# mj129/Tramba

Hardware: AMD Instinct MI355X
Metric: images/sec fwd Tramba-V 384x384 (higher is better)
Workload: dtype bf16; 1 GPU; Tramba-V (VMamba-B encoder) 384x384 bf16 inference, batch 4 per GPU, random-init weights (seed 1026), randn images; global_batch=4, launch=hipGraph replay, decoder guide branches on a side stream

## Files before the change

### include/tramba_hip.h

```cpp
#ifndef TRAMBA_HIP_H
#define TRAMBA_HIP_H

#include <stddef.h>
#include <stdint.h>

#ifdef __cplusplus
extern "C" {
#endif

typedef enum { TRAMBA_F32 = 0, TRAMBA_F16 = 1, TRAMBA_BF16 = 2 } tramba_dtype;

typedef enum {
    TRAMBA_SCAN_RASTER = 0,
    TRAMBA_SCAN_LINE = 1,
    TRAMBA_SCAN_HELIX = 2,
    TRAMBA_SCAN_WINDOW = 3,
    TRAMBA_SCAN_DILATION = 4
} tramba_scan_family;

typedef enum { TRAMBA_ACT_NONE = 0, TRAMBA_ACT_SILU = 1, TRAMBA_ACT_GELU = 2,
               TRAMBA_ACT_SIGMOID_GATE = 3 ,
               TRAMBA_ACT_GELU_GRAD_MUL = 4
             } tramba_act;

// ... 133 lines not shown
                     int64_t m, int n, int k, int act, int dtype, int out_dtype, void *stream);
int tramba_linear_ln_cl(const void *x, const void *w_folded, const float *colsum, const float *bias, const void *residual,
                        void *y, int64_t m, int n, int k, float eps, int act, int dtype, int out_dtype, void *stream);
int tramba_linear2_cl(const void *x1, const void *x2, int k1, const void *w, const float *bias, const void *residual,
                      void *y, int64_t m, int n, int k, int act, int dtype, int out_dtype, void *stream);

int tramba_linear_dual_cl(const void *x, const void *w, const float *bias, void *y_pre, void *y_act, int64_t m, int n,
                          int k, int act, int dtype, void *stream);
size_t tramba_wgrad_workspace(int64_t m, int n, int k, int groups, int nbatch);
int tramba_wgrad_cl(const void *gy, const void *x, float *out, void *workspace, size_t workspace_bytes, int64_t m, int n,
                    int k, int groups, int nbatch, int64_t gy_bs, int64_t gy_gs, int gy_ld, int64_t x_bs, int64_t x_gs,
                    int x_ld, int want_bias, int dtype, void *stream);
int tramba_wgrad_parts_cl(const void *gy, const void *x, float *out, void *workspace, size_t workspace_bytes, int64_t m,
                          int n, int k, int groups, int nbatch, int64_t gy_bs, int64_t gy_gs, int gy_ld, int64_t x_bs,
                          int64_t x_gs, int x_ld, int want_bias, int dtype, void *stream, int *nslab);
int tramba_rows_gemm_cl(const void *x, const void *w, float *y, int nz, int64_t m, int n, int k, int groups, int ldy,
                        int dtype, void *stream);
int tramba_shadow_cast_multi(const void *table, int ntensors, int64_t total_tiles, int dtype, void *stream);
int tramba_slab_sum(const float *part, float *out, int64_t n, int nslab, void *stream);
int tramba_multi_sum_strided(const float *const *parts, float *const *outs, const int64_t *n, const int64_t *stride,
                             const int *nslab, int count, void *stream);
int tramba_multi_sum(const float *const *parts, float *const *outs, const int64_t *n, const int *nslab, int count,
                     void *stream);

int tramba_expand_norm_head_cl(const void *x, const void *w, const float *ln_w, const float *ln_b,
                               const float *head_w, float head_b, float *y, int batch, int h, int wd, int cin, int p,
                               float eps, int dtype, void *stream);

int tramba_conv3x3s2_cl(const void *x, const void *w, const float *bias, void *y, int batch, int hin,
                        int win, int cin, int cout, int dtype, void *stream);
int tramba_stem_conv_ln_gelu(const void *img, const float *w, const float *bias, const float *ln_w,
                             const float *ln_b, void *y, int batch, int h, int wd, float eps,
                             int img_dtype, int dtype, void *stream);

#define TRAMBA_EVAL_NINT 520
#define TRAMBA_EVAL_NDBL 48
int tramba_saliency_stats(const float *pred, const unsigned char *gt, long long *ints, double *dbl, int batch, int h,
                          int w, void *stream);
#define TRAMBA_WFM_MAX_DIM 4096
int tramba_feature_transform(const unsigned char *gt, int *idx, int *dist2, int batch, int h, int w, void *stream);
size_t tramba_weighted_f_workspace(int batch, int h, int w);
int tramba_weighted_f_sums(const float *pred, const unsigned char *gt, const int *idx, const int *dist2, const double *gauss,
                           double *sums, void *workspace, size_t workspace_bytes, int batch, int h, int w, void *stream);

#define TRAMBA_FRAME_MAX_DIM 16384
#define TRAMBA_FRAME_MAX_OUT 2048
size_t tramba_resize_table_words(int in_h, int in_w, int out_h, int out_w);
int tramba_resize_table(int in_h, int in_w, int out_h, int out_w, const double *mean, const double *std, int *table,
                        size_t words);
int tramba_frames_to_input(const unsigned char *frames, const int *table, float *out, int batch, int h, int w, int out_h,
                           int out_w, int bgr, void *stream);
int tramba_logits_to_u8(const void *logits, unsigned char *out, int batch, int in_h, int in_w, int h, int w, int dtype,
                        void *stream);
#define TRAMBA_FRAMES_DESC_WORDS 16
#define TRAMBA_RAGGED_IN 1
#define TRAMBA_RAGGED_OUT 2
int tramba_frames_ragged_check(const int64_t *desc_host, int batch, int size, size_t packed_bytes, size_t out_capacity,
                               int parts);
int tramba_frames_to_input_ragged(const unsigned char *packed, const int64_t *desc_host, size_t packed_bytes, float *out,
                                  int batch, int size, int bgr, void *stream);
int tramba_logits_to_u8_ragged(const void *logits, const unsigned char *packed, const int64_t *desc_host, unsigned char *out,
                               size_t out_capacity, int batch, int size, int dtype, void *stream);

#define TRAMBA_AUG_DESC_WORDS 32
#define TRAMBA_AUG_CONTRAST 0
#define TRAMBA_AUG_BRIGHTNESS 1
// ... 102 lines not shown
```

### tramba_amd/csrc/norm_conv.hip

```cpp
#include <stdlib.h>
#include <string.h>

#include "common.h"
#include "norm.h"

namespace tramba {

template <typename T, int V>
__global__ __launch_bounds__(256) void layernorm_cl_kernel(const T *__restrict__ x,
                                                          const float *__restrict__ w,
                                                          const float *__restrict__ bvec, T *__restrict__ y,
                                                          long rows, int C, float eps, int act, int P, int H,
                                                          int W)
{
    const int lane = threadIdx.x & (kWave - 1);
    const long row = (long)blockIdx.x * (blockDim.x >> 6) + __builtin_amdgcn_readfirstlane(threadIdx.x >> 6);
    if (row >= rows) return;
    const int nit = (C + kWave * V - 1) / (kWave * V);
    float acc[kNormMaxIt][V];
    const T *xr = x + row * C;
#pragma unroll
    for (int it = 0; it < kNormMaxIt; ++it) {
#pragma unroll
        for (int v = 0; v < V; ++v) acc[it][v] = 0.f;
// ... 1033 lines not shown
                    dw_v2f p[TW];
#pragma unroll
                    for (int t = 0; t < TW; ++t) {
                        p[t] = acc[u % KS][t];
                        acc[u % KS][t] = bias;
                    }
                    if constexpr (DUAL) {
#pragma unroll
                        for (int t = 0; t < TW; ++t) {
                            dw_store2<T>(rp, voff[t + R], so, p[t]);
                            p[t] = dw_v2f{Cvt<T>::to_f(Cvt<T>::from_f(p[t].x)), Cvt<T>::to_f(Cvt<T>::from_f(p[t].y))};
                        }
                    }
                    if (act == TRAMBA_ACT_GELU) {
#pragma unroll
                        for (int t = 0; t < TW; ++t) p[t] = dw_v2f{geluf_(p[t].x), geluf_(p[t].y)};
                    } else if (act == TRAMBA_ACT_SILU) {
#pragma unroll
                        for (int t = 0; t < TW; ++t) p[t] = dw_v2f{siluf_(p[t].x), siluf_(p[t].y)};
                    }
#pragma unroll
                    for (int t = 0; t < TW; ++t) dw_store2<T>(ry, voff[t + R], so, p[t]);
                }
                issue(q + D < nq ? r + D : -1, swr);
                srd = srd + 1 == NS ? 0 : srd + 1;
                swr = swr + 1 == NS ? 0 : swr + 1;
            }
        }
    }
    asm volatile("s_waitcnt vmcnt(0)" ::: "memory");
#endif
}

template <typename T>
__device__ __forceinline__ dw_v2f dw_load2(__amdgpu_buffer_rsrc_t r, unsigned voff)
{
    if constexpr (sizeof(T) == 4) {
        return __builtin_bit_cast(dw_v2f, __builtin_amdgcn_raw_buffer_load_b64(r, voff, 0, 0));
    } else {
        const unsigned raw = __builtin_amdgcn_raw_buffer_load_b32(r, voff, 0, 0);
        const Pack<T, 2> pk = __builtin_bit_cast(Pack<T, 2>, raw);
        return dw_v2f{Cvt<T>::to_f(pk.v[0]), Cvt<T>::to_f(pk.v[1])};
    }
}

constexpr int dwg_waves(int ks) { return ks <= 3 ? 16 : 8; }

template <typename T, int KS>
__global__ __launch_bounds__(dwg_waves(KS) * kWave) void dwconv_wgrad_cl_kernel(const T *__restrict__ x,
                                                                          const T *__restrict__ gy,
                                                                          float *__restrict__ part, int H, int W, int C,
                                                                          int RPW, int CS)
{
    constexpr int V = 2, R = KS / 2, TW = 4, NI = TW + KS - 1, kDwgWaves = dwg_waves(KS);
    __shared__ float red[KS * KS + 1][2 * kWave];
    const int lane = threadIdx.x & (kWave - 1);
    const int wv = __builtin_amdgcn_readfirstlane(threadIdx.x >> 6);
    const int c0 = (blockIdx.x * kWave + lane) * V;
    const bool cok = c0 + V <= C;
    const int band = blockIdx.y / CS, cs = blockIdx.y % CS;
    const int row0 = (band * kDwgWaves + wv) * RPW;
    const int wseg = ((W + CS - 1) / CS + TW - 1) / TW * TW;
    const int wlo = cs * wseg, whi = wlo + wseg < W ? wlo + wseg : W;
    const int b = blockIdx.z;
    const unsigned colb = (unsigned)C * (unsigned)sizeof(T), rowb = (unsigned)W * colb;
    const __amdgpu_buffer_rsrc_t rx = make_rsrc(x + (long)b * H * W * C, (unsigned)H * rowb);
// ... 254 lines not shown
    return TRAMBA_OK;
}

static int dw7_band_rows(long items4, int H)
{
    const int cand[] = {6, 8, 12, 16, 24, 32, 48, 64, 96, 128, 192};
    int best = H;
    double best_cost = 1e30;
    for (int th : cand) {
        if (th > H && th != cand[0]) continue;
        const int t = th > H ? H : th;
        const long nwg = items4 * ((H + t - 1) / t);
        const double cost = (double)((nwg + 255) / 256) * (t * 196.0 + (t + 6) * 50.0 + 150.0);
        if (cost < best_cost) { best_cost = cost; best = t; }
    }
    return best;
}

template <typename T>
static int launch_dw7_march(const void *x, const float *wt, const float *bt, void *y, int B, int H, int W, int C, int act,
                            hipStream_t s, void *ypre, int flip)
{
    const int nct = (C / 2 + 63) / 64, ncg = (W + kDwmTW - 1) / kDwmTW;
    const long items4 = ((long)nct * ncg * B + 3) / 4;
    int th = dw7_band_rows(items4, H);
    const int forced = tramba_tune_get(TRAMBA_TUNE_DW_ROWS);
    if (forced > 0) th = forced > H ? H : forced;
    const int nbands = (H + th - 1) / th;
    if (ypre)
        hipLaunchKernelGGL((dwconv7_march_kernel<T, true>), dim3((unsigned)(items4 * nbands)), dim3(256), 0, s, (const T *)x, wt, bt,
                           (T *)y, B, H, W, C, act, (T *)ypre, flip, th, nbands, nct, ncg);
    else
        hipLaunchKernelGGL((dwconv7_march_kernel<T, false>), dim3((unsigned)(items4 * nbands)), dim3(256), 0, s, (const T *)x, wt, bt,
                           (T *)y, B, H, W, C, act, (T *)ypre, flip, th, nbands, nct, ncg);
    TRAMBA_LAUNCH_CHECK();
    return TRAMBA_OK;
}

}

using namespace tramba;

extern "C" int tramba_layernorm_cl(const void *x, const float *w, const float *b, void *y, int64_t rows,
                                   int c, float eps, int act, int dtype, void *stream)
{
    TRAMBA_CHECK(x && w && b && y, "layernorm_cl: null tensor");
    TRAMBA_CHECK(rows > 0 && c > 0, "layernorm_cl: empty shape");
    TRAMBA_CHECK(aligned16(x) && aligned16(y), "layernorm_cl: tensors must be 16-byte aligned");
    ProfScope prof(TRAMBA_PROF_LAYERNORM, (hipStream_t)stream, 2.0 * (double)rows * c * dtype_size(dtype));
    TRAMBA_DISPATCH_DTYPE(dtype, T,
        return launch_layernorm<T>(x, w, b, y, rows, c, eps, act, 1, 1, 1, (hipStream_t)stream));
    return TRAMBA_OK;
}

static long ln_bwd_rows_per_wave(long rows, bool rows_form)
{
    long rpw = rows / 4096;
    const long lo = rows_form ? 4 : 2;
    return rpw < lo ? lo : (rpw > 128 ? 128 : rpw);
}

static bool ln_bwd_rows_form(int c, int dtype)
{
    const int vm = dtype == TRAMBA_F32 ? 4 : 8;
    return c % vm == 0 && c <= kWave * vm;
}
// ... 451 lines not shown
        constexpr int VM = 16 / (int)sizeof(T);
        if (vec) {
            const long total = pixels * (c / VM);
            hipLaunchKernelGGL((col2im3x3_cl_kernel<T, VM>), dim3((unsigned)((total + 255) / 256)), dim3(256), 0, s,
                               (const T *)gcols, (T *)gx, h, wd, c, ho, wo, stride, pad, ckp, total);
        } else {
            const long total = pixels * c;
            hipLaunchKernelGGL((col2im3x3_cl_kernel<T, 1>), dim3((unsigned)((total + 255) / 256)), dim3(256), 0, s,
                               (const T *)gcols, (T *)gx, h, wd, c, ho, wo, stride, pad, ckp, total);
        }
    });
    TRAMBA_LAUNCH_CHECK();
    return TRAMBA_OK;
}

extern "C" int tramba_dwconv_cl(const void *x, const float *wt, const float *bt, void *y, int batch, int h,
                                int wd, int c, int ks, int act, int dtype, void *stream)
{
    return tramba_dwconv_dual_cl(x, wt, bt, nullptr, y, batch, h, wd, c, ks, act, 0, dtype, stream);
}

extern "C" int tramba_dwconv_dual_cl(const void *x, const float *wt, const float *bt, void *y_pre, void *y, int batch,
                                     int h, int wd, int c, int ks, int act, int flip_taps, int dtype, void *stream)
{
    TRAMBA_CHECK(x && wt && bt && y, "dwconv_cl: null tensor");
    TRAMBA_CHECK(!y_pre || aligned16(y_pre), "dwconv_cl: tensors must be 16-byte aligned");
    TRAMBA_CHECK(batch > 0 && h > 0 && wd > 0 && c > 0, "dwconv_cl: empty shape");
    TRAMBA_CHECK(ks == 3 || ks == 5 || ks == 7, "dwconv_cl: kernel size %d unsupported (3,5,7)", ks);
    TRAMBA_CHECK(aligned16(x) && aligned16(y) && aligned16(wt) && aligned16(bt), "dwconv_cl: tensors must be 16-byte aligned");
    hipStream_t s = (hipStream_t)stream;
    ProfScope prof(TRAMBA_PROF_DW, s, (y_pre ? 3.0 : 2.0) * (double)batch * h * wd * c * dtype_size(dtype));
    const bool march = ks == 7 && c % 8 == 0 && tramba_tune_get(TRAMBA_TUNE_DW_FORM) != 1 &&
                       (double)h * wd * c * 4.0 < 2147483648.0 && (double)batch * wd * c < 2147483648.0;
    TRAMBA_DISPATCH_DTYPE(dtype, T, {
        if (march) return launch_dw7_march<T>(x, wt, bt, y, batch, h, wd, c, act, s, y_pre, flip_taps);
        if (ks == 3) return launch_dw<T, 3>(x, wt, bt, y, batch, h, wd, c, act, s, y_pre, flip_taps);
        if (ks == 5) return launch_dw<T, 5>(x, wt, bt, y, batch, h, wd, c, act, s, y_pre, flip_taps);
        return launch_dw<T, 7>(x, wt, bt, y, batch, h, wd, c, act, s, y_pre, flip_taps);
    });
    return TRAMBA_OK;
}
```

### tramba_amd/csrc/stem.hip

```cpp
#include "common.h"

namespace tramba {

constexpr int kStemCout = 64, kStemTaps = 27;

template <typename TI, typename T>
__global__ __launch_bounds__(256) void stem_conv_ln_gelu_kernel(const TI *__restrict__ img, const float *__restrict__ w,
                                                               const float *__restrict__ bias,
                                                               const float *__restrict__ ln_w,
                                                               const float *__restrict__ ln_b, T *__restrict__ y,
                                                               int B, int H, int W, int Ho, int Wo, float eps)
{
    __shared__ __attribute__((aligned(16))) float wl[kStemTaps][kStemCout];
    for (int t = threadIdx.x; t < kStemTaps * kStemCout; t += blockDim.x) {
        const int co = t / kStemTaps, tap = t % kStemTaps;
        wl[tap][co] = w[t];
    }
    __syncthreads();
    const long pix = (long)blockIdx.x * 64 + (threadIdx.x >> 2);
    const int part = threadIdx.x & 3;
    const long npix = (long)B * Ho * Wo;
    const bool ok = pix < npix;
    const long pp = ok ? pix : npix - 1;
    const int wo = (int)(pp % Wo);
    const long t2 = pp / Wo;
    const int ho = (int)(t2 % Ho), b = (int)(t2 / Ho);

    float acc[16];
#pragma unroll
    for (int j = 0; j < 16; ++j) acc[j] = bias[part * 16 + j];
#pragma unroll 1
    for (int ci = 0; ci < 3; ++ci)
#pragma unroll 1
        for (int ky = 0; ky < 3; ++ky) {
            const int hy = 2 * ho + ky - 1;
#pragma unroll
            for (int kx = 0; kx < 3; ++kx) {
                const int wx = 2 * wo + kx - 1;
                float v = 0.f;
                if (hy >= 0 && hy < H && wx >= 0 && wx < W) v = Cvt<TI>::to_f(img[(((long)b * 3 + ci) * H + hy) * W + wx]);
                const float4 *wp = reinterpret_cast<const float4 *>(&wl[ci * 9 + ky * 3 + kx][part * 16]);
#pragma unroll
                for (int q = 0; q < 4; ++q) {
                    const float4 ww = wp[q];
                    acc[4 * q + 0] = fmaf(v, ww.x, acc[4 * q + 0]);
                    acc[4 * q + 1] = fmaf(v, ww.y, acc[4 * q + 1]);
                    acc[4 * q + 2] = fmaf(v, ww.z, acc[4 * q + 2]);
                    acc[4 * q + 3] = fmaf(v, ww.w, acc[4 * q + 3]);
                }
            }
        }
    float s = 0.f;
#pragma unroll
    for (int j = 0; j < 16; ++j) s += acc[j];
    s += __shfl_xor(s, 1, 4);
    s += __shfl_xor(s, 2, 4);
    const float mean = s * (1.f / kStemCout);
    float q2 = 0.f;
#pragma unroll
    for (int j = 0; j < 16; ++j) {
        const float d = acc[j] - mean;
        q2 = fmaf(d, d, q2);
    }
    q2 += __shfl_xor(q2, 1, 4);
    q2 += __shfl_xor(q2, 2, 4);
    const float rstd = rsqrtf(q2 * (1.f / kStemCout) + eps);
    if (!ok) return;
    T *yo = y + pix * kStemCout + part * 16;
#pragma unroll
    for (int h8 = 0; h8 < 2; ++h8) {
        float o[8];
#pragma unroll
        for (int j = 0; j < 8; ++j) {
            const int c = part * 16 + h8 * 8 + j;
            o[j] = geluf_((acc[h8 * 8 + j] - mean) * rstd * ln_w[c] + ln_b[c]);
        }
        store_pack<T, 8>(yo + h8 * 8, o);
    }
}

}

using namespace tramba;

extern "C" int tramba_stem_conv_ln_gelu(const void *img, const float *w, const float *bias, const float *ln_w,
                                        const float *ln_b, void *y, int batch, int h, int wd, float eps,
                                        int img_dtype, int dtype, void *stream)
{
    TRAMBA_CHECK(img && w && bias && ln_w && ln_b && y, "stem_conv_ln_gelu: null tensor");
    TRAMBA_CHECK(batch > 0 && h > 0 && wd > 0, "stem_conv_ln_gelu: empty shape");
    TRAMBA_CHECK(img_dtype == TRAMBA_F32 || img_dtype == dtype, "stem_conv_ln_gelu: image must be f32 or the activation dtype");
    TRAMBA_CHECK(aligned16(y), "stem_conv_ln_gelu: output must be 16-byte aligned");
    const int ho = (h + 1) / 2, wo = (wd + 1) / 2;
    const long npix = (long)batch * ho * wo;
    dim3 grid((unsigned)((npix + 63) / 64)), block(256);
    hipStream_t s = (hipStream_t)stream;
    TRAMBA_DISPATCH_DTYPE(dtype, T, {
        if (img_dtype == TRAMBA_F32 && dtype != TRAMBA_F32)
            hipLaunchKernelGGL((stem_conv_ln_gelu_kernel<float, T>), grid, block, 0, s, (const float *)img, w, bias, ln_w,
                               ln_b, (T *)y, batch, h, wd, ho, wo, eps);
        else
            hipLaunchKernelGGL((stem_conv_ln_gelu_kernel<T, T>), grid, block, 0, s, (const T *)img, w, bias, ln_w, ln_b,
                               (T *)y, batch, h, wd, ho, wo, eps);
    });
    TRAMBA_LAUNCH_CHECK();
    return TRAMBA_OK;
}
```

### tramba_amd/hip.py

```python
import ctypes
import os
import threading
import weakref

import numpy as np
import torch

_HERE = os.path.dirname(os.path.abspath(__file__))
LIB_PATH = os.path.join(_HERE, "_lib", "libtramba_hip.so")

F32, F16, BF16 = 0, 1, 2
ACT_NONE, ACT_SILU, ACT_GELU, ACT_SIGMOID_GATE, ACT_GELU_GRAD_MUL = 0, 1, 2, 3, 4
SCAN_RASTER, SCAN_LINE, SCAN_HELIX, SCAN_WINDOW, SCAN_DILATION = range(5)
FAMILY = {"raster": SCAN_RASTER, "line": SCAN_LINE, "helix": SCAN_HELIX, "window": SCAN_WINDOW,
          "dilation": SCAN_DILATION}
PROF_SCAN_BOUNDARY, PROF_SCAN_FUSED, PROF_GEMM, PROF_MERGE, PROF_SCAN_BWD, PROF_WGRAD, PROF_LAYERNORM, PROF_DW = 0, 1, 2, 3, 4, 5, 6, 7

_DT = {torch.float32: F32, torch.float16: F16, torch.bfloat16: BF16}

c_int, c_i64, c_f, c_vp = ctypes.c_int, ctypes.c_int64, ctypes.c_float, ctypes.c_void_p

SIGNATURES = {
    "tramba_last_error": (ctypes.c_char_p, []),
    "tramba_abi_version": (c_int, []),
# ... 53 lines not shown
    "tramba_augment_scale_taps": (c_int, [c_int] * 2),
    "tramba_augment_rotation": (c_int, [c_int] * 2 + [c_vp]),
    "tramba_augment_workspace": (ctypes.c_size_t, [c_int] * 2),
    "tramba_augment_batch": (c_int, [c_vp] * 2 + [ctypes.c_size_t] + [c_vp] * 4 + [ctypes.c_size_t] + [c_int] * 2 + [c_vp]),
    "tramba_dw_pack": (c_int, [c_vp] * 8 + [c_int] * 2 + [c_vp]),
    "tramba_dwconv_cl": (c_int, [c_vp] * 4 + [c_int] * 7 + [c_vp]),
    "tramba_dwconv_dual_cl": (c_int, [c_vp] * 5 + [c_int] * 8 + [c_vp]),
    "tramba_dw_unpack_grad": (c_int, [c_vp] * 5 + [c_int] * 3 + [c_vp]),
    "tramba_dw_pack_multi": (c_int, [c_vp] * 10 + [c_int, c_vp]),
    "tramba_dw_unpack_grad_multi": (c_int, [c_vp] * 8 + [c_int, c_vp]),
    "tramba_im2col3x3_cl": (c_int, [c_vp] * 2 + [c_int] * 8 + [c_vp]),
    "tramba_upsample_bilinear_bwd": (c_int, [c_vp] * 2 + [c_int] * 5 + [c_vp]),
    "tramba_col2im3x3_cl": (c_int, [c_vp] * 2 + [c_int] * 8 + [c_vp]),
    "tramba_dwconv_wgrad_parts": (c_i64, [c_int, c_int, c_int, c_int, c_int]),
    "tramba_dwconv_wgrad_cl": (c_int, [c_vp] * 3 + [c_int] * 6 + [c_vp]),
    "tramba_dct_split_cl": (c_int, [c_vp] * 6 + [c_int] * 4 + [c_vp]),
    "tramba_linear_cl": (c_int, [c_vp] * 5 + [c_i64, c_int, c_int, c_int, c_int, c_int, c_vp]),
    "tramba_linear_dual_cl": (c_int, [c_vp] * 5 + [c_i64, c_int, c_int, c_int, c_int, c_vp]),
    "tramba_linear_ln_cl": (c_int, [c_vp] * 6 + [c_i64, c_int, c_int, c_f, c_int, c_int, c_int, c_vp]),
    "tramba_linear2_cl": (c_int, [c_vp, c_vp, c_int] + [c_vp] * 4 + [c_i64, c_int, c_int, c_int, c_int, c_int, c_vp]),
    "tramba_wgrad_workspace": (ctypes.c_size_t, [c_i64, c_int, c_int, c_int, c_int]),
    "tramba_wgrad_cl": (c_int, [c_vp] * 4 + [ctypes.c_size_t, c_i64, c_int, c_int, c_int, c_int, c_i64, c_i64, c_int, c_i64,
                                             c_i64, c_int, c_int, c_int, c_vp]),
    "tramba_rows_gemm_cl": (c_int, [c_vp] * 3 + [c_int, c_i64, c_int, c_int, c_int, c_int, c_int, c_vp]),
    "tramba_shadow_cast_multi": (c_int, [c_vp, c_int, c_i64, c_int, c_vp]),
    "tramba_slab_sum": (c_int, [c_vp, c_vp, c_i64, c_int, c_vp]),
    "tramba_multi_sum": (c_int, [c_vp, c_vp, c_vp, c_vp, c_int, c_vp]),
    "tramba_multi_sum_strided": (c_int, [c_vp, c_vp, c_vp, c_vp, c_vp, c_int, c_vp]),
    "tramba_wgrad_parts_cl": (c_int, [c_vp] * 4 + [ctypes.c_size_t, c_i64, c_int, c_int, c_int, c_int, c_i64, c_i64, c_int, c_i64,
                                                   c_i64, c_int, c_int, c_int, c_vp, c_vp]),
    "tramba_expand_norm_head_cl": (c_int, [c_vp] * 5 + [c_f, c_vp] + [c_int] * 5 + [c_f, c_int, c_vp]),
    "tramba_conv3x3s2_cl": (c_int, [c_vp] * 4 + [c_int] * 6 + [c_vp]),
    "tramba_stem_conv_ln_gelu": (c_int, [c_vp] * 6 + [c_int] * 3 + [c_f, c_int, c_int, c_vp]),
    "tramba_sod_loss_sums": (c_int, [c_vp] * 3 + [c_int] * 6 + [c_vp]),
    "tramba_sod_loss_finish": (c_int, [c_vp] * 4 + [c_int, c_int, c_i64, c_vp, c_vp]),
    "tramba_sod_loss_grad_workspace": (ctypes.c_size_t, [c_int] * 5),
    "tramba_sod_loss_grad": (c_int, [c_vp] * 6 + [ctypes.c_size_t] + [c_int] * 5 + [c_vp]),
    "tramba_loss_weight_map": (c_int, [c_vp] * 2 + [c_int] * 4 + [c_vp]),
    "tramba_sod_wloss_sums": (c_int, [c_vp] * 4 + [c_int] * 6 + [c_f, c_int, c_vp]),
    "tramba_sod_wloss_finish": (c_int, [c_vp] * 4 + [c_int, c_int, c_i64, c_int, c_int, c_vp, c_vp]),
    "tramba_sod_wloss_grad_workspace": (ctypes.c_size_t, [c_int] * 5),
    "tramba_sod_wloss_grad": (c_int, [c_vp] * 7 + [ctypes.c_size_t] + [c_int] * 5 + [c_f, c_int, c_vp]),
    "tramba_adam_step": (c_int, [c_vp] * 6 + [c_int] + [ctypes.c_double] * 5 + [c_vp]),
    "tramba_grad_accumulate": (c_int, [c_vp] * 3 + [c_int, c_vp, c_vp]),
    "tramba_grad_norm_workspace": (ctypes.c_size_t, [c_vp, c_int]),
    "tramba_grad_norm": (c_int, [c_vp] * 2 + [c_int, ctypes.c_double, ctypes.c_double, c_int, c_vp, c_vp, ctypes.c_size_t, c_vp]),
    "tramba_adam_step_ctl": (c_int, [c_vp] * 6 + [c_int] + [ctypes.c_double] * 5 + [c_vp] * 3),
    "tramba_window_attn_cl": (c_int, [c_vp] * 3 + [c_int] * 8 + [c_vp]),
    "tramba_kv_attn_cl": (c_int, [c_vp] * 3 + [c_int, c_i64] + [c_int] * 4 + [c_vp]),
    "tramba_window_attn_bwd_work": (ctypes.c_size_t, [c_int] * 6),
    "tramba_window_attn_bwd_cl": (c_int, [c_vp] * 6 + [ctypes.c_size_t] + [c_int] * 8 + [c_vp]),
    "tramba_kv_attn_bwd_work": (ctypes.c_size_t, [c_int, c_i64, c_int, c_int, c_int]),
    "tramba_kv_attn_bwd_cl": (c_int, [c_vp] * 6 + [ctypes.c_size_t, c_int, c_i64] + [c_int] * 4 + [c_vp]),
    "tramba_patch_conv_cl": (c_int, [c_vp] * 4 + [c_int] * 7 + [c_vp]),
    "tramba_patch_conv_dgrad_cl": (c_int, [c_vp] * 3 + [c_int] * 7 + [c_vp]),
    "tramba_patch_conv_wgrad_split": (c_int, [c_int] * 6),
    "tramba_patch_conv_wgrad_work": (ctypes.c_size_t, [c_int] * 6),
    "tramba_patch_conv_wgrad_cl": (c_int, [c_vp] * 3 + [ctypes.c_size_t] + [c_int] * 8 + [c_vp]),
    "tramba_patch_embed_ln": (c_int, [c_vp] * 6 + [c_int] * 7 + [c_f, c_int, c_int, c_vp]),
    "tramba_conv_affine_cl": (c_int, [c_vp] * 6 + [c_int] * 9 + [c_vp]),
    "tramba_stem7_affine_relu_pool": (c_int, [c_vp] * 5 + [c_int] * 5 + [c_vp]),
    "tramba_conv_dgrad_cl": (c_int, [c_vp] * 3 + [c_int] * 8 + [c_vp]),
    "tramba_conv_wgrad_split": (c_int, [c_int] * 7),
    "tramba_conv_wgrad_work": (ctypes.c_size_t, [c_int] * 7),
    "tramba_conv_wgrad_cl": (c_int, [c_vp] * 3 + [ctypes.c_size_t] + [c_int] * 8 + [c_vp]),
    "tramba_bn_parts": (c_int, [c_i64, c_int]),
# ... 1416 lines not shown
    nslab = part.shape[0]
    n = part.numel() // max(nslab, 1)
    if part.dtype != torch.float32 or not part.is_contiguous() or n % 4 or nslab == 0:
        return part.sum(dim=0)
    out = torch.empty(part.shape[1:], dtype=torch.float32, device=part.device)
    if defer and _sumq.enabled:
        if _sumq.poison:
            out.fill_(float("nan"))
        _enqueue_sum(_ptr(part), _ptr(out), n, nslab, (part, out))
        return out
    _check(lib().tramba_slab_sum(_ptr(part), _ptr(out), n, nslab, _stream()), "slab_sum")
    return out


def shadow_cast_multi(table, ntensors, total_tiles, dtype):
    _dev(table)
    if table.dtype != torch.int64 or table.shape != (ntensors, 8) or not table.is_contiguous():
        raise TrambaHipError("shadow_cast_multi: table must be a contiguous (ntensors, 8) int64 tensor")
    _check(lib().tramba_shadow_cast_multi(_ptr(table), ntensors, total_tiles, _DT[dtype], _stream()), "shadow_cast_multi")


def conv3x3s2_cl(x, w_kmajor, bias):
    _dev(x, w_kmajor, bias)
    bb, h, wd, cin = x.shape
    cout = w_kmajor.shape[0]
    if w_kmajor.dtype != x.dtype or w_kmajor.shape[1] != 9 * cin:
        raise TrambaHipError("conv3x3s2_cl: weight dtype/shape mismatch")
    y = torch.empty((bb, (h + 1) // 2, (wd + 1) // 2, cout), dtype=x.dtype, device=x.device)
    _check(lib().tramba_conv3x3s2_cl(_ptr(x), _ptr(w_kmajor), _ptr(bias), _ptr(y), bb, h, wd, cin, cout, dt(x),
                                     _stream()), "conv3x3s2_cl")
    return y


def stem_conv_ln_gelu(img, w, bias, ln_w, ln_b, eps, out_dtype):
    _dev(img, w, bias, ln_w, ln_b)
    bb, c3, h, wd = img.shape
    if c3 != 3 or tuple(w.shape) != (64, 3, 3, 3):
        raise TrambaHipError("stem_conv_ln_gelu: expects a 3 -> 64 channel 3x3 stem")
    y = torch.empty((bb, (h + 1) // 2, (wd + 1) // 2, 64), dtype=out_dtype, device=img.device)
    _check(lib().tramba_stem_conv_ln_gelu(_ptr(img), _ptr(w), _ptr(bias), _ptr(ln_w), _ptr(ln_b), _ptr(y), bb, h, wd,
                                          eps, _DT[img.dtype], _DT[out_dtype], _stream()), "stem_conv_ln_gelu")
    return y


_PATCH_EMBED_FORMS = ((7, 4, 3, 64), (4, 4, 0, 128))


def patch_conv_supported(dtype, cin, cout, r):
    return dtype in _ATTN_DTYPES and 2 <= r <= 8 and cin > 0 and cin % 64 == 0 and cout > 0 and cout % 8 == 0


def patch_conv_cl(x, w_kmajor, bias):
    _dev(x, w_kmajor, bias)
    if x.dim() != 4 or w_kmajor.dim() != 4 or w_kmajor.dtype != x.dtype or w_kmajor.shape[1] != w_kmajor.shape[2] \
            or w_kmajor.shape[3] != x.shape[3]:
        raise TrambaHipError(f"patch_conv_cl: need x (B, H, W, Cin) and w (Cout, r, r, Cin) of one dtype, got {tuple(x.shape)} "
                             f"{x.dtype} {tuple(w_kmajor.shape)} {w_kmajor.dtype}")
    bb, h, wd, cin = x.shape
    cout, r = w_kmajor.shape[0], w_kmajor.shape[1]
    if bias is not None and (bias.dtype != torch.float32 or tuple(bias.shape) != (cout,)):
        raise TrambaHipError(f"patch_conv_cl: bias must be float32 ({cout},)")
    if (bb * h * wd * cin * 2) >= 2 ** 31:
        raise TrambaHipError("patch_conv_cl: input map beyond 32-bit byte offsets")
    y = torch.empty((bb, h // max(r, 1), wd // max(r, 1), cout), dtype=x.dtype, device=x.device)
    _check(lib().tramba_patch_conv_cl(_ptr(x), _ptr(w_kmajor), _ptr(bias), _ptr(y), bb, h, wd, cin, cout, r, dt(x), _stream()),
           "patch_conv_cl")
    return y


def patch_conv_train_supported(dtype, cin, cout, r):
    return patch_conv_supported(dtype, cin, cout, r) and cout * r * r * cin * 4 < 2 ** 31


def _patch_conv_geom(name, gy, x_shape, x_dtype):
# ... 286 lines not shown
```

### tramba_amd/models.py

```python
from collections import OrderedDict

import torch
import torch.nn as nn
import torch.nn.functional as F

from . import hip
from .modules import (FinalPatchExpand_X4, FreqBlockv6, LayerNorm2d, Linear2d, MultiScaleDecoderBlock, PatchExpand,
                      VSSMEncoder, _cache, _infer, _init_weights, _run_blocks, model_mask_pool, _need_device, from_cl,
                      load_pretrained_Base, to_cl)
from .ops import CrossMerge_Line, CrossScan_Line


OVERLAP_BRANCHES = True
OVERLAP_TRAINING = True
_side_streams = {}


def _side_stream(device):
    key = str(device)
    st = _side_streams.get(key)
    if st is None:
        st = _side_streams[key] = torch.cuda.Stream(device=device)
    return st

# ... 115 lines not shown
        n = len(self.stage_layers)
        for s in range(n):
            if s == n - 1:
                outs.append(self._final_cl(x_low))
                break
            x = self.expand_layers[s]._forward_cl(x_low)
            if s < n - 1:
                if guides is not None and s in guides:
                    mid, ready = guides[s]
                    torch.cuda.current_stream().wait_event(ready)
                    mid.record_stream(torch.cuda.current_stream())
                    if torch.is_grad_enabled() and mid.requires_grad:
                        mid = _StreamEdge.apply(mid, _side_stream(mid.device))
                else:
                    mid = self.guide_layers[s]._forward_cl(skips_cl[-(s + 2)])
                x = self.concat_back_dim[s]._forward_cat_cl(x, mid)
                x = _run_blocks(self.stage_layers[s].blocks, x)
            if self.deep_supervision or s == n - 1:
                outs.append(self._seg_cl(self.seg_layers[s], x))
            x_low = x
        return outs if self.deep_supervision else outs[0]

    def forward(self, skips):
        return self._forward_cl([skips[0]] + [to_cl(s) for s in skips[1:]])


class BaseUMamba(nn.Module):

    def __init__(self, vss_args, decoder_args, use_pretrain=True, pretrained_path=""):
        super().__init__()
        self.vssm_encoder = VSSMEncoder(**vss_args)
        self.decoder = VSSMDecoder(**decoder_args)
        self.compute_dtype = None
        if use_pretrain:
            load_pretrained_Base(self.vssm_encoder, ckpt_path=pretrained_path)

    def _forward_overlapped(self, x):
        main = torch.cuda.current_stream()
        side = _side_stream(x.device)
        dec = self.decoder
        n = len(dec.stage_layers)
        guides = {}

        def on_stage(i, feat):
            s = n - 2 - i
            if s < 0 or s >= len(dec.guide_layers):
                return
            if (torch.is_grad_enabled() and _OVERLAP_TRAINING_STAGES is not None and s not in _OVERLAP_TRAINING_STAGES) or (
                    not torch.is_grad_enabled() and _OVERLAP_INFER_STAGES is not None and s not in _OVERLAP_INFER_STAGES):
                return
            side.wait_stream(main)
            feat.record_stream(side)
            with torch.cuda.stream(side):
                fin = _StreamEdge.apply(feat, main) if torch.is_grad_enabled() and feat.requires_grad else feat
                mid = dec.guide_layers[s]._forward_cl(fin)
                ready = torch.cuda.Event()
                ready.record(side)
            guides[s] = (mid, ready)

        skips = self.vssm_encoder._forward_cl(x, on_stage=on_stage)
        out = dec._forward_cl(skips, guides=guides)
        main.wait_stream(side)
        return out

    def forward(self, x):
        _need_device(x)
        if self.training:
            model_mask_pool(self).begin_step()
        if self.compute_dtype is not None:
            x = x.to(self.compute_dtype)
        if OVERLAP_BRANCHES and (OVERLAP_TRAINING or not torch.is_grad_enabled()) and type(self.decoder) is VSSMDecoder:
            out = self._forward_overlapped(x)
        else:
            skips = self.vssm_encoder._forward_cl(x)
            out = self.decoder._forward_cl(skips)
        if self.compute_dtype is not None:
            out = [o.float() for o in out] if isinstance(out, list) else out.float()
        return out

    @torch.no_grad()
    def freeze_encoder(self):
        for name, p in self.vssm_encoder.named_parameters():
            if "patch_embed" not in name:
                p.requires_grad = False

    @torch.no_grad()
    def unfreeze_encoder(self):
        for p in self.vssm_encoder.parameters():
            p.requires_grad = True


def bulid_model(deep_supervision=True, use_pretrain=True, img_size=384, dims=128, depths=[2, 2, 2, 2],
                pretrained_path=""):
    vss_args = dict(patch_size=4, in_chans=3, depths=[2, 2, 15, 2], dims=dims, drop_path_rate=0.6, patch_norm=True,
                    norm_layer="LN2D", posembed=False, imgsize=img_size)
    decoder_args = dict(deep_supervision=deep_supervision, features_per_stage=[dims, dims * 2, dims * 4, dims * 8],
                        depths=depths, img_size=img_size, drop_path_rate=0.2)
    return BaseUMamba(vss_args, decoder_args, use_pretrain=use_pretrain, pretrained_path=pretrained_path)


def _bn_affine(bn: nn.BatchNorm2d, dtype=torch.float32):
    var, mean = bn.running_var.detach().to(dtype), bn.running_mean.detach().to(dtype)
    scale = 1.0 / torch.sqrt(var + bn.eps)
    if bn.weight is not None:
        scale = bn.weight.detach().to(dtype) * scale
    shift = -mean * scale
    if bn.bias is not None:
# ... 264 lines not shown
```

### tramba_amd/modules.py

```python
import math
from collections import OrderedDict

import torch
import torch.nn as nn
import torch.nn.functional as F

from . import hip
from .ops import (CrossMerge, CrossMerge_Dilation, CrossMerge_Line, CrossMerge_Window, CrossScan,
                  CrossScan_Dilation, CrossScan_Line, CrossScan_Window, SelectiveScanOflex)



FOLD_LAYERNORM = True


def to_cl(x: torch.Tensor) -> torch.Tensor:
    return x.permute(0, 2, 3, 1).contiguous()


def from_cl(x: torch.Tensor) -> torch.Tensor:
    return x.permute(0, 3, 1, 2)


def _need_device(x):
# ... 1702 lines not shown

    def __init__(self, patch_size=4, in_chans=3, depths=[2, 2, 15, 2], dims=128, drop_path_rate=0.6,
                 patch_norm=True, norm_layer="LN2D", posembed=False, imgsize=224, **kwargs):
        super().__init__()
        assert norm_layer.lower() == "ln2d" and patch_norm and not posembed
        self.channel_first = True
        self.num_layers = len(depths)
        if isinstance(dims, int):
            dims = [int(dims * 2 ** i) for i in range(self.num_layers)]
        self.num_features = dims[-1]
        self.dims = dims
        dpr = [x.item() for x in torch.linspace(0, drop_path_rate, sum(depths))]
        self.pos_embed = None
        stride = patch_size // 2
        self.patch_embed = nn.Sequential(
            nn.Conv2d(in_chans, dims[0] // 2, kernel_size=stride + 1, stride=stride, padding=1),
            nn.Identity(), LayerNorm2d(dims[0] // 2), nn.Identity(), nn.GELU(),
            nn.Conv2d(dims[0] // 2, dims[0], kernel_size=stride + 1, stride=stride, padding=1),
            nn.Identity(), LayerNorm2d(dims[0]))
        self.layers = nn.ModuleList()
        self.downsample = nn.ModuleList()
        for i in range(self.num_layers):
            if i < self.num_layers - 1:
                self.downsample.append(nn.Sequential(
                    nn.Identity(), nn.Conv2d(dims[i], dims[i] * 2, kernel_size=3, stride=2, padding=1),
                    nn.Identity(), LayerNorm2d(dims[i] * 2)))
            else:
                self.downsample.append(nn.Identity())
            blocks = [VSSBlock(hidden_dim=dims[i], drop_path=dp, norm_layer=LayerNorm2d, channel_first=True)
                      for dp in dpr[sum(depths[:i]):sum(depths[:i + 1])]]
            self.layers.append(nn.Sequential(OrderedDict(blocks=nn.Sequential(*blocks))))
        self.apply(_init_weights)

    def _forward_cl(self, x_img, on_stage=None):
        feats = [x_img]
        pe = self.patch_embed
        if (_infer(x_img, pe[0].weight) and pe[0].in_channels == 3 and pe[0].out_channels == 64
                and pe[0].kernel_size == (3, 3) and pe[0].stride == (2, 2) and x_img.is_contiguous()):
            act_dtype = pe[5].weight.dtype if pe[5].weight.dtype != torch.float32 else x_img.dtype
            x = hip.stem_conv_ln_gelu(x_img, _f32(pe[0].weight), _f32(pe[0].bias), _f32(pe[2].weight),
                                      _f32(pe[2].bias), pe[2].eps, act_dtype)
        else:
            x = _conv_cl(pe[0], to_cl(x_img))
            x = pe[2]._forward_cl(x, act=hip.ACT_GELU)
        x = _conv_cl(pe[5], x)
        x = pe[7]._forward_cl(x)
        for s, layer in enumerate(self.layers):
            x = _run_blocks(layer.blocks, x)
            feats.append(x)
            if on_stage is not None:
                on_stage(s, x)
            if s < self.num_layers - 1:
                ds = self.downsample[s]
                x = ds[3]._forward_cl(_conv_cl(ds[1], x))
        return feats

    def forward(self, x):
        _need_device(x)
        feats = self._forward_cl(x)
        return [feats[0]] + [from_cl(f) for f in feats[1:]]


def load_pretrained_Base(model, ckpt_path=""):
    import re
    print(f"Loading weights from: {ckpt_path}")
    ckpt = torch.load(ckpt_path, map_location="cpu")
    model_dict = model.state_dict()
    loaded = set()
    for k, v in ckpt["model"].items():
        if "classifier" in k:
            print(f"Passing weights: {k}")
            continue
        if "downsample" in k:
            i_ds = int(re.findall(r"layers\.(\d+)\.downsample", k)[0])
            k = k.replace(f"layers.{i_ds}.downsample", f"downsample.{i_ds}")
# ... 16 lines not shown
```

Before: 874.6 img/s.

## Add register-marching 3x3 depthwise conv kernel and fuse image cast into stem

Adds a row-marching depthwise 3x3 kernel that keeps a ring of input rows in registers and sliding accumulators. It is dispatched for ks=3 when channel occupancy pays off. Separately, the fp32-to-bf16 image cast is folded into the stem conv kernel by rounding the inputs in registers, which removes a standalone cast kernel. The new dw kernel adds band-size heuristics and a code path whose speed depends on channel count.

New measurement: 880.1 img/s (median of 6 runs). No clear change (+0.6%).

```diff
diff --git a/include/tramba_hip.h b/include/tramba_hip.h
--- a/include/tramba_hip.h
+++ b/include/tramba_hip.h
@@ -189,6 +189,9 @@
 int tramba_stem_conv_ln_gelu(const void *img, const float *w, const float *bias, const float *ln_w,
                              const float *ln_b, void *y, int batch, int h, int wd, float eps,
                              int img_dtype, int dtype, void *stream);
+int tramba_stem_conv_ln_gelu_rounded(const void *img, const float *w, const float *bias, const float *ln_w,
+                                     const float *ln_b, void *y, int batch, int h, int wd, float eps,
+                                     int img_dtype, int dtype, void *stream);
 
 #define TRAMBA_EVAL_NINT 520
 #define TRAMBA_EVAL_NDBL 48
diff --git a/tramba_amd/csrc/norm_conv.hip b/tramba_amd/csrc/norm_conv.hip
--- a/tramba_amd/csrc/norm_conv.hip
+++ b/tramba_amd/csrc/norm_conv.hip
@@ -1089,6 +1089,120 @@
 #endif
 }
 
+template <typename T, bool DUAL>
+__global__ __launch_bounds__(256) void dwconv3_march_kernel(const T *__restrict__ x, const float *__restrict__ wt,
+                                                           const float *__restrict__ bt, T *__restrict__ y, int B, int H,
+                                                           int W, int C, int act, T *__restrict__ ypre, int flip, int TH,
+                                                           int nbands, int nct, int ncg)
+{
+    constexpr int KS = 3, R = 1, TW = kDwmTW, NI = TW + KS - 1, D = 2, NS = D + 1;
+    static_assert(NS == KS, "the row loop is unrolled once for the accumulator window and the register ring");
+    const unsigned lin = blockIdx.x, nblk = gridDim.x;
+    const unsigned q8 = nblk >> 3, r8 = nblk & 7, xcd = lin & 7, slot8 = lin >> 3;
+    const unsigned t_ = xcd * q8 + (xcd < r8 ? xcd : r8) + slot8;
+    const unsigned band = t_ % (unsigned)nbands, iblk = t_ / (unsigned)nbands;
+    const int wave = __builtin_amdgcn_readfirstlane(threadIdx.x >> 6), lane = threadIdx.x & 63;
+    const unsigned item = iblk * 4u + (unsigned)wave;
+    if (item >= (unsigned)(nct * ncg * B)) return;
+    const int ct = (int)(item % (unsigned)nct);
+    const int cgp = (int)((item / (unsigned)nct) % (unsigned)ncg);
+    const int b = (int)(item / (unsigned)(nct * ncg));
+    const int c0 = (ct * 64 + lane) * 2;
+    const bool cok = c0 + 2 <= C;
+    const int w0 = cgp * TW;
+    const int h0 = (int)band * TH, hend = h0 + TH < H ? h0 + TH : H;
+
+    const unsigned colb = (unsigned)C * (unsigned)sizeof(T), rowb = (unsigned)W * colb;
+    const T *const xb = x + (long)b * H * W * C;
+    const __amdgpu_buffer_rsrc_t ry = make_rsrc(y + (long)b * H * W * C, (unsigned)H * rowb);
+    const __amdgpu_buffer_rsrc_t rp = make_rsrc(DUAL ? ypre + (long)b * H * W * C : y, DUAL ? (unsigned)H * rowb : 0u);
+    const __amdgpu_buffer_rsrc_t rw = make_rsrc(wt, (unsigned)(KS * KS) * (unsigned)C * 4u);
+
+    unsigned voff[NI];
+#pragma unroll
+    for (int i = 0; i < NI; ++i) {
+        const int wx = w0 - R + i;
+        voff[i] = (cok && wx >= 0 && wx < W) ? (unsigned)(wx * C + c0) * (unsigned)sizeof(T) : kOutOfRange;
+    }
+    auto issue = [&](int r, DwRaw2<T> (&dst)[NI]) {
+        const bool ok = r >= 0 && r < H;
+        const __amdgpu_buffer_rsrc_t rr = make_rsrc(xb, ok ? (unsigned)H * rowb : 0u);
+        const unsigned so = ok ? (unsigned)r * rowb : 0u;
+#pragma unroll
+        for (int i = 0; i < NI; ++i) dst[i] = dw_load2_raw<T>(rr, voff[i], so);
+    };
+    DwRaw2<T> raw[NS][NI];
+    issue(h0 - R, raw[0]);
+    issue(h0 - R + 1, raw[1]);
+    dw_v2f wv[KS * KS];
+    {
+        const unsigned wo = cok ? (unsigned)c0 * 4u : kOutOfRange;
+#pragma unroll
+        for (int i = 0; i < KS * KS; ++i)
+            wv[i] = __builtin_bit_cast(dw_v2f, __builtin_amdgcn_raw_buffer_load_b64(
+                                                   rw, wo, (unsigned)(flip ? KS * KS - 1 - i : i) * (unsigned)C * 4u, 0));
+    }
+    dw_v2f bias = {0.f, 0.f};
+    if (cok) bias = dw_v2f{bt[c0], bt[c0 + 1]};
+    dw_v2f acc[KS][TW];
+#pragma unroll
+    for (int sl = 0; sl < KS; ++sl)
+#pragma unroll
+        for (int t = 0; t < TW; ++t) acc[sl][t] = bias;
+
+    const int nq = (hend - h0) + KS - 1;
+    for (int qb = 0; qb < nq; qb += KS) {
+#pragma unroll
+        for (int u = 0; u < KS; ++u) {
+            const int q = qb + u;
+            if (q < nq) {
+                const int r = h0 - R + q;
+                issue(q + D < nq ? r + D : -1, raw[(u + D) % NS]);
+                dw_v2f xin[NI];
+#pragma unroll
+                for (int i = 0; i < NI; ++i) xin[i] = dw_cvt2<T>(raw[u][i]);
+#pragma unroll
+                for (int dy = 0; dy < KS; ++dy) {
+                    const int o = r + R - dy;
+                    if (o >= h0 && o < hend) {
+                        const int sl = (u + KS - dy) % KS;
+#pragma unroll
+                        for (int dx = 0; dx < KS; ++dx)
+#pragma unroll
+                            for (int t = 0; t < TW; ++t) acc[sl][t] = xin[t + dx] * wv[dy * KS + dx] + acc[sl][t];
+                    }
+                }
+                if (q >= KS - 1) {
+                    const int sl = (u + 1) % KS;
+                    const unsigned so = (unsigned)(r - R) * rowb;
+                    dw_v2f p[TW];
+#pragma unroll
+                    for (int t = 0; t < TW; ++t) {
+                        p[t] = acc[sl][t];
+                        acc[sl][t] = bias;
+                    }
+                    if constexpr (DUAL) {
+#pragma unroll
+                        for (int t = 0; t < TW; ++t) {
+                            dw_store2<T>(rp, voff[t + R], so, p[t]);
+                            p[t] = dw_v2f{Cvt<T>::to_f(Cvt<T>::from_f(p[t].x)), Cvt<T>::to_f(Cvt<T>::from_f(p[t].y))};
+                        }
+                    }
+                    if (act == TRAMBA_ACT_GELU) {
+#pragma unroll
+                        for (int t = 0; t < TW; ++t) p[t] = dw_v2f{geluf_(p[t].x), geluf_(p[t].y)};
+                    } else if (act == TRAMBA_ACT_SILU) {
+#pragma unroll
+                        for (int t = 0; t < TW; ++t) p[t] = dw_v2f{siluf_(p[t].x), siluf_(p[t].y)};
+                    }
+#pragma unroll
+                    for (int t = 0; t < TW; ++t) dw_store2<T>(ry, voff[t + R], so, p[t]);
+                }
+            }
+        }
+    }
+}
+
 template <typename T>
 __device__ __forceinline__ dw_v2f dw_load2(__amdgpu_buffer_rsrc_t r, unsigned voff)
 {
@@ -1409,6 +1523,47 @@
                            (T *)y, B, H, W, C, act, (T *)ypre, flip, th, nbands, nct, ncg);
     else
         hipLaunchKernelGGL((dwconv7_march_kernel<T, false>), dim3((unsigned)(items4 * nbands)), dim3(256), 0, s, (const T *)x, wt, bt,
+                           (T *)y, B, H, W, C, act, (T *)ypre, flip, th, nbands, nct, ncg);
+    TRAMBA_LAUNCH_CHECK();
+    return TRAMBA_OK;
+}
+
+static int dw3_band_rows(long items4, int H)
+{
+    const int cand[] = {2, 3, 4, 6, 8, 12, 16, 24, 32, 48, 64, 96, 128, 192};
+    int best = H;
+    double best_cost = 1e30;
+    for (int th : cand) {
+        if (th > H && th != cand[0]) continue;
+        const int t = th > H ? H : th;
+        const long nwg = items4 * ((H + t - 1) / t);
+        const double cost = (double)((nwg + 255) / 256) * (t * 160.0 + 2 * 45.0 + 120.0);
+        if (cost < best_cost) { best_cost = cost; best = t; }
+    }
+    return best;
+}
+
+static bool dw3_march_pays(int C)
+{
+    const int nct = (C / 2 + 63) / 64;
+    return (C / 2) * 4 >= nct * 64 * 3;
+}
+
+template <typename T>
+static int launch_dw3_march(const void *x, const float *wt, const float *bt, void *y, int B, int H, int W, int C, int act,
+                            hipStream_t s, void *ypre, int flip)
+{
+    const int nct = (C / 2 + 63) / 64, ncg = (W + kDwmTW - 1) / kDwmTW;
+    const long items4 = ((long)nct * ncg * B + 3) / 4;
+    int th = dw3_band_rows(items4, H);
+    const int forced = tramba_tune_get(TRAMBA_TUNE_DW_ROWS);
+    if (forced > 0) th = forced > H ? H : forced;
+    const int nbands = (H + th - 1) / th;
+    if (ypre)
+        hipLaunchKernelGGL((dwconv3_march_kernel<T, true>), dim3((unsigned)(items4 * nbands)), dim3(256), 0, s, (const T *)x, wt, bt,
+                           (T *)y, B, H, W, C, act, (T *)ypre, flip, th, nbands, nct, ncg);
+    else
+        hipLaunchKernelGGL((dwconv3_march_kernel<T, false>), dim3((unsigned)(items4 * nbands)), dim3(256), 0, s, (const T *)x, wt, bt,
                            (T *)y, B, H, W, C, act, (T *)ypre, flip, th, nbands, nct, ncg);
     TRAMBA_LAUNCH_CHECK();
     return TRAMBA_OK;
@@ -1926,8 +2081,14 @@
     ProfScope prof(TRAMBA_PROF_DW, s, (y_pre ? 3.0 : 2.0) * (double)batch * h * wd * c * dtype_size(dtype));
     const bool march = ks == 7 && c % 8 == 0 && tramba_tune_get(TRAMBA_TUNE_DW_FORM) != 1 &&
                        (double)h * wd * c * 4.0 < 2147483648.0 && (double)batch * wd * c < 2147483648.0;
+    const int form = tramba_tune_get(TRAMBA_TUNE_DW_FORM);
+    const bool can3 = ks == 3 && c % 4 == 0 && (act == TRAMBA_ACT_NONE || act == TRAMBA_ACT_SILU || act == TRAMBA_ACT_GELU) &&
+                      (double)h * wd * c * 4.0 < 2147483648.0 && (double)batch * wd * c < 2147483648.0 &&
+                      (double)batch * wd * c / 8.0 * h < 2147483648.0;
+    const bool march3 = can3 && form != 1 && (form == 2 || dw3_march_pays(c));
     TRAMBA_DISPATCH_DTYPE(dtype, T, {
         if (march) return launch_dw7_march<T>(x, wt, bt, y, batch, h, wd, c, act, s, y_pre, flip_taps);
+        if (march3) return launch_dw3_march<T>(x, wt, bt, y, batch, h, wd, c, act, s, y_pre, flip_taps);
         if (ks == 3) return launch_dw<T, 3>(x, wt, bt, y, batch, h, wd, c, act, s, y_pre, flip_taps);
         if (ks == 5) return launch_dw<T, 5>(x, wt, bt, y, batch, h, wd, c, act, s, y_pre, flip_taps);
         return launch_dw<T, 7>(x, wt, bt, y, batch, h, wd, c, act, s, y_pre, flip_taps);
diff --git a/tramba_amd/csrc/stem.hip b/tramba_amd/csrc/stem.hip
--- a/tramba_amd/csrc/stem.hip
+++ b/tramba_amd/csrc/stem.hip
@@ -4,7 +4,7 @@
 
 constexpr int kStemCout = 64, kStemTaps = 27;
 
-template <typename TI, typename T>
+template <typename TI, typename T, bool ROUND = false>
 __global__ __launch_bounds__(256) void stem_conv_ln_gelu_kernel(const TI *__restrict__ img, const float *__restrict__ w,
                                                                const float *__restrict__ bias,
                                                                const float *__restrict__ ln_w,
@@ -39,6 +39,7 @@
                 const int wx = 2 * wo + kx - 1;
                 float v = 0.f;
                 if (hy >= 0 && hy < H && wx >= 0 && wx < W) v = Cvt<TI>::to_f(img[(((long)b * 3 + ci) * H + hy) * W + wx]);
+                if constexpr (ROUND) v = Cvt<T>::to_f(Cvt<T>::from_f(v));
                 const float4 *wp = reinterpret_cast<const float4 *>(&wl[ci * 9 + ky * 3 + kx][part * 16]);
 #pragma unroll
                 for (int q = 0; q < 4; ++q) {
@@ -83,9 +84,8 @@
 
 using namespace tramba;
 
-extern "C" int tramba_stem_conv_ln_gelu(const void *img, const float *w, const float *bias, const float *ln_w,
-                                        const float *ln_b, void *y, int batch, int h, int wd, float eps,
-                                        int img_dtype, int dtype, void *stream)
+static int stem_launch(const void *img, const float *w, const float *bias, const float *ln_w, const float *ln_b, void *y,
+                       int batch, int h, int wd, float eps, int img_dtype, int dtype, bool round_img, void *stream)
 {
     TRAMBA_CHECK(img && w && bias && ln_w && ln_b && y, "stem_conv_ln_gelu: null tensor");
     TRAMBA_CHECK(batch > 0 && h > 0 && wd > 0, "stem_conv_ln_gelu: empty shape");
@@ -96,7 +96,10 @@
     dim3 grid((unsigned)((npix + 63) / 64)), block(256);
     hipStream_t s = (hipStream_t)stream;
     TRAMBA_DISPATCH_DTYPE(dtype, T, {
-        if (img_dtype == TRAMBA_F32 && dtype != TRAMBA_F32)
+        if (img_dtype == TRAMBA_F32 && dtype != TRAMBA_F32 && round_img)
+            hipLaunchKernelGGL((stem_conv_ln_gelu_kernel<float, T, true>), grid, block, 0, s, (const float *)img, w, bias, ln_w,
+                               ln_b, (T *)y, batch, h, wd, ho, wo, eps);
+        else if (img_dtype == TRAMBA_F32 && dtype != TRAMBA_F32)
             hipLaunchKernelGGL((stem_conv_ln_gelu_kernel<float, T>), grid, block, 0, s, (const float *)img, w, bias, ln_w,
                                ln_b, (T *)y, batch, h, wd, ho, wo, eps);
         else
@@ -106,3 +109,17 @@
     TRAMBA_LAUNCH_CHECK();
     return TRAMBA_OK;
 }
+
+extern "C" int tramba_stem_conv_ln_gelu(const void *img, const float *w, const float *bias, const float *ln_w,
+                                        const float *ln_b, void *y, int batch, int h, int wd, float eps,
+                                        int img_dtype, int dtype, void *stream)
+{
+    return stem_launch(img, w, bias, ln_w, ln_b, y, batch, h, wd, eps, img_dtype, dtype, false, stream);
+}
+
+extern "C" int tramba_stem_conv_ln_gelu_rounded(const void *img, const float *w, const float *bias, const float *ln_w,
+                                                const float *ln_b, void *y, int batch, int h, int wd, float eps,
+                                                int img_dtype, int dtype, void *stream)
+{
+    return stem_launch(img, w, bias, ln_w, ln_b, y, batch, h, wd, eps, img_dtype, dtype, true, stream);
+}
diff --git a/tramba_amd/hip.py b/tramba_amd/hip.py
--- a/tramba_amd/hip.py
+++ b/tramba_amd/hip.py
@@ -109,6 +109,7 @@
     "tramba_expand_norm_head_cl": (c_int, [c_vp] * 5 + [c_f, c_vp] + [c_int] * 5 + [c_f, c_int, c_vp]),
     "tramba_conv3x3s2_cl": (c_int, [c_vp] * 4 + [c_int] * 6 + [c_vp]),
     "tramba_stem_conv_ln_gelu": (c_int, [c_vp] * 6 + [c_int] * 3 + [c_f, c_int, c_int, c_vp]),
+    "tramba_stem_conv_ln_gelu_rounded": (c_int, [c_vp] * 6 + [c_int] * 3 + [c_f, c_int, c_int, c_vp]),
     "tramba_sod_loss_sums": (c_int, [c_vp] * 3 + [c_int] * 6 + [c_vp]),
     "tramba_sod_loss_finish": (c_int, [c_vp] * 4 + [c_int, c_int, c_i64, c_vp, c_vp]),
     "tramba_sod_loss_grad_workspace": (ctypes.c_size_t, [c_int] * 5),
@@ -1591,14 +1592,15 @@
     return y
 
 
-def stem_conv_ln_gelu(img, w, bias, ln_w, ln_b, eps, out_dtype):
+def stem_conv_ln_gelu(img, w, bias, ln_w, ln_b, eps, out_dtype, round_input=False):
     _dev(img, w, bias, ln_w, ln_b)
     bb, c3, h, wd = img.shape
     if c3 != 3 or tuple(w.shape) != (64, 3, 3, 3):
         raise TrambaHipError("stem_conv_ln_gelu: expects a 3 -> 64 channel 3x3 stem")
     y = torch.empty((bb, (h + 1) // 2, (wd + 1) // 2, 64), dtype=out_dtype, device=img.device)
-    _check(lib().tramba_stem_conv_ln_gelu(_ptr(img), _ptr(w), _ptr(bias), _ptr(ln_w), _ptr(ln_b), _ptr(y), bb, h, wd,
-                                          eps, _DT[img.dtype], _DT[out_dtype], _stream()), "stem_conv_ln_gelu")
+    entry = lib().tramba_stem_conv_ln_gelu_rounded if round_input else lib().tramba_stem_conv_ln_gelu
+    _check(entry(_ptr(img), _ptr(w), _ptr(bias), _ptr(ln_w), _ptr(ln_b), _ptr(y), bb, h, wd,
+                 eps, _DT[img.dtype], _DT[out_dtype], _stream()), "stem_conv_ln_gelu")
     return y
 
 
diff --git a/tramba_amd/models.py b/tramba_amd/models.py
--- a/tramba_amd/models.py
+++ b/tramba_amd/models.py
@@ -171,10 +171,11 @@
         self.vssm_encoder = VSSMEncoder(**vss_args)
         self.decoder = VSSMDecoder(**decoder_args)
         self.compute_dtype = None
+        self.fused_input_cast = True
         if use_pretrain:
             load_pretrained_Base(self.vssm_encoder, ckpt_path=pretrained_path)
 
-    def _forward_overlapped(self, x):
+    def _forward_overlapped(self, x, cast_image=None):
         main = torch.cuda.current_stream()
         side = _side_stream(x.device)
         dec = self.decoder
@@ -197,7 +198,7 @@
                 ready.record(side)
             guides[s] = (mid, ready)
 
-        skips = self.vssm_encoder._forward_cl(x, on_stage=on_stage)
+        skips = self.vssm_encoder._forward_cl(x, on_stage=on_stage, cast_image=cast_image)
         out = dec._forward_cl(skips, guides=guides)
         main.wait_stream(side)
         return out
@@ -206,12 +207,17 @@
         _need_device(x)
         if self.training:
             model_mask_pool(self).begin_step()
+        cast_image = None
         if self.compute_dtype is not None:
-            x = x.to(self.compute_dtype)
+            if (self.fused_input_cast and x.dtype == torch.float32 and self.compute_dtype != torch.float32
+                    and not self.training and not torch.is_grad_enabled()):
+                cast_image = self.compute_dtype
+            else:
+                x = x.to(self.compute_dtype)
         if OVERLAP_BRANCHES and (OVERLAP_TRAINING or not torch.is_grad_enabled()) and type(self.decoder) is VSSMDecoder:
-            out = self._forward_overlapped(x)
+            out = self._forward_overlapped(x, cast_image)
         else:
-            skips = self.vssm_encoder._forward_cl(x)
+            skips = self.vssm_encoder._forward_cl(x, cast_image=cast_image)
             out = self.decoder._forward_cl(skips)
         if self.compute_dtype is not None:
             out = [o.float() for o in out] if isinstance(out, list) else out.float()
diff --git a/tramba_amd/modules.py b/tramba_amd/modules.py
--- a/tramba_amd/modules.py
+++ b/tramba_amd/modules.py
@@ -1758,15 +1758,18 @@
             self.layers.append(nn.Sequential(OrderedDict(blocks=nn.Sequential(*blocks))))
         self.apply(_init_weights)
 
-    def _forward_cl(self, x_img, on_stage=None):
+    def _forward_cl(self, x_img, on_stage=None, cast_image=None):
         feats = [x_img]
         pe = self.patch_embed
         if (_infer(x_img, pe[0].weight) and pe[0].in_channels == 3 and pe[0].out_channels == 64
-                and pe[0].kernel_size == (3, 3) and pe[0].stride == (2, 2) and x_img.is_contiguous()):
+                and pe[0].kernel_size == (3, 3) and pe[0].stride == (2, 2) and x_img.is_contiguous()
+                and (cast_image is None or pe[5].weight.dtype == cast_image)):
             act_dtype = pe[5].weight.dtype if pe[5].weight.dtype != torch.float32 else x_img.dtype
             x = hip.stem_conv_ln_gelu(x_img, _f32(pe[0].weight), _f32(pe[0].bias), _f32(pe[2].weight),
-                                      _f32(pe[2].bias), pe[2].eps, act_dtype)
+                                      _f32(pe[2].bias), pe[2].eps, act_dtype, round_input=cast_image is not None)
         else:
+            if cast_image is not None:
+                x_img = x_img.to(cast_image)
             x = _conv_cl(pe[0], to_cl(x_img))
             x = pe[2]._forward_cl(x, act=hip.ACT_GELU)
         x = _conv_cl(pe[5], x)
```
